# YinkaiYu/Hybrid-Monte-Carlo-for-d-wave-SC

Hardware: AMD Instinct MI355X
Metric: fp64 leapfrog steps/sec at L=32, 1→8 MI355X; % fp64 MFMA roofline (higher is better)
Workload: dtype f64; 1 GPU; L=32 beta=16 single-chain HMC (BASELINE configs[2], C3); L=32, N=1024, bdg_dim=2048, chains_per_gpu=1, Nt=7, therm_sweeps=100, poles=12, parallelism=single GPU

## Files before the change

hybrid-monte-carlo-for-d-wave-sc_amd/csrc/dwhmc_cr_sparse.hip:

```cpp
#include "dwhmc_device.h"
#include "dwhmc_internal.h"

namespace dwh {
namespace {

__device__ __forceinline__ void cmac(double2& a, double2 b, double2 c) {
  a.x = fma(b.x, c.x, fma(-b.y, c.y, a.x));
  a.y = fma(b.x, c.y, fma(b.y, c.x, a.y));
}
__device__ __forceinline__ void rmac(double2& a, double s, double2 c) {
  a.x = fma(s, c.x, a.x);
  a.y = fma(s, c.y, a.y);
}

__device__ __forceinline__ double sp_flip(double x, unsigned m) {
  return __builtin_bit_cast(double, __builtin_bit_cast(unsigned long long, x) ^ ((unsigned long long)m << 32));
}

__device__ __forceinline__ double sp_uniform(double x) {
  const unsigned long long b = __builtin_bit_cast(unsigned long long, x);
  const unsigned lo = __builtin_amdgcn_readfirstlane((unsigned)b), hi = __builtin_amdgcn_readfirstlane((unsigned)(b >> 32));
  return __builtin_bit_cast(double, (unsigned long long)hi << 32 | lo);
}

// ... 6 lines not shown
    crot = cb < HB ? cb + HB : cb - HB;
    mx = cb >= HB ? 0x80000000u : 0u;
    my = cb < HB ? 0x80000000u : 0u;
  }
  __device__ __forceinline__ double2 ld(const double2* base, unsigned row) const {
    return *reinterpret_cast<const double2*>(reinterpret_cast<const char*>(base) + (row + crot));
  }
  __device__ __forceinline__ double2 sign(double2 u) const {
    return make_double2(sp_flip(u.x, mx), sp_flip(u.y, my));
  }
};

__device__ __forceinline__ double2 sp_cval(double2 x, int m) {
  if ((m & 0x3fffff) == 0) return x;
  const int op = (m >> 22) & 3;
  return make_double2(op == 2 ? -0.5 * x.x : 0.5 * x.x, op == 0 ? 0.5 * x.y : -0.5 * x.y);
}

constexpr int kSpRowsWG = 4;
constexpr int NZ = kCrSpNZ, NH = kCrSpNZ - 1;
#ifndef SP_WAVES_F
#define SP_WAVES_F 6
#endif
#ifndef SP_WAVES_B
#define SP_WAVES_B 6
#endif
#ifndef SP_RPW_B
#define SP_RPW_B 1
#endif
template <int BP>
constexpr int kSpWavesF = BP <= 64 ? SP_WAVES_F : 2;
template <int BP>
constexpr int kSpWavesB = BP <= 64 ? SP_WAVES_B : 2;

__device__ __forceinline__ void wave_sync() {
  __builtin_amdgcn_fence(__ATOMIC_RELEASE, "wavefront");
  __builtin_amdgcn_wave_barrier();
  __builtin_amdgcn_fence(__ATOMIC_ACQUIRE, "wavefront");
}

__device__ __forceinline__ double2 sp_ld(const double2* base, unsigned off) {
  return *reinterpret_cast<const double2*>(reinterpret_cast<const char*>(base) + off);
}
__device__ __forceinline__ void sp_st(double2* base, unsigned off, double2 v) {
  *reinterpret_cast<double2*>(reinterpret_cast<char*>(base) + off) = v;
}

template <int BP, int NB>
struct ColStage {
  static constexpr int TOT = NB * NZ * BP, IT = (TOT + 64 * kSpRowsWG - 1) / (64 * kSpRowsWG);
  int m[IT];
  double2 x[IT];
  __device__ __forceinline__ void load_meta(const int* __restrict__ tcm) {
#pragma unroll
    for (int i = 0; i < IT; ++i) m[i] = tcm[min((int)threadIdx.x + 64 * kSpRowsWG * i, TOT - 1)];
  }
  __device__ __forceinline__ void load_values(const double2* __restrict__ tcv, const double2* __restrict__ Dc) {
#pragma unroll
    for (int i = 0; i < IT; ++i) {
      const int q = min((int)threadIdx.x + 64 * kSpRowsWG * i, TOT - 1), s = m[i] & 0x3fffff;
      x[i] = *(s ? Dc + (s - 1) : tcv + q);
    }
  }
  __device__ __forceinline__ void pin_meta() {
#pragma unroll
    for (int i = 0; i < IT; ++i) asm volatile("" : "+v"(m[i]));
// ... 159 lines not shown
#pragma unroll
          for (int e = 0; e < NH; ++e) gh[o][g][e][j] = sp_ld(base, t.ho[o][g][e] + cl[j]);
          gp[o][g][j] = bc.ld(base, t.po[o][g]);
        }
    }
    __builtin_amdgcn_sched_barrier(0);
    double2 yk[NCL][2];
#pragma unroll
    for (int j = 0; j < NCL; ++j) {
      const BotCol<BP> bc(cl[j]);
      double2 ya = make_double2(0.0, 0.0), yc = ya;
#pragma unroll
      for (int o = 0; o < 2; ++o) {
#pragma unroll
        for (int e = 0; e < NH; ++e) {
          rmac(ya, t.hv[o][e], gh[o][0][e][j]);
          rmac(yc, t.hv[o][e], gh[o][1][e][j]);
        }
        cmac(ya, pw[o], bc.sign(gp[o][0][j]));
        cmac(yc, pw[o], bc.sign(gp[o][1][j]));
      }
      yk[j][0] = ya;
      yk[j][1] = yc;
    }
#pragma unroll
    for (int j = 0; j < NCL; ++j)
      asm volatile("" : "+v"(yk[j][0].x), "+v"(yk[j][0].y), "+v"(yk[j][1].x), "+v"(yk[j][1].y));
    __builtin_amdgcn_sched_barrier(0);
    __syncthreads();
    if (i == 0) {
      cs.finish(cv, ci);
      __syncthreads();
    }
#pragma unroll
    for (int j = 0; j < NCL; ++j) {
      const int c = cl[j] / sizeof(double2);
      double2 za = make_double2(0.0, 0.0), zc = za;
#pragma unroll
      for (int e = 0; e < NZ; ++e) {
        const double2 wa = cv[0][e][c], we = cv[1][e][c];
        const unsigned ka = ci[0][e][c], ke = ci[1][e][c];
        cmac(za, sp_ld(gr[w][0], ka), wa);
        cmac(zc, sp_ld(gr[w][1], ka), wa);
        cmac(za, sp_ld(gr[w][2], ke), we);
        cmac(zc, sp_ld(gr[w][3], ke), we);
      }
      if (l + 64 * j < BP) {
        sp_st(base, t.oya + cl[j], yk[j][0]);
        sp_st(base, t.oyc + cl[j], yk[j][1]);
        sp_st(base, t.oza + cl[j], za);
        sp_st(base, t.ozc + cl[j], zc);
      }
    }
    wave_sync();
#pragma unroll
    for (int j = 0; j < NCL; ++j)
      if (l + 64 * j < BP) {
        sp_st(sc[w][0], cl[j], yk[j][0]);
        sp_st(sc[w][1], cl[j], yk[j][1]);
      }
    wave_sync();
#pragma unroll
    for (int j = 0; j < NCL; ++j) {
      const int c = cl[j] / sizeof(double2);
      double2 mx = make_double2(0.0, 0.0);
#pragma unroll
      for (int e = 0; e < NZ; ++e) {
        cmac(mx, sp_ld(sc[w][0], ci[0][e][c]), cv[0][e][c]);
        cmac(mx, sp_ld(sc[w][1], ci[1][e][c]), cv[1][e][c]);
      }
      if (l + 64 * j < BP) sp_st(base, t.omx + cl[j], mx);
    }
    if (RPW > 1) wave_sync();
  }
}

}

void launch_cr_sp_fwd(const CrDims& c, double2* pool, const CrSpRowFwd* recs, int n, const double2* tcv,
                      const int* tcm, const double2* Delta, hipStream_t s) {
  if (n <= 0) return;
  const dim3 g(n * (c.BP / 2 / kSpRowsWG), c.nbatch), b(64 * kSpRowsWG);
  switch (c.BP) {
    case 32: hipLaunchKernelGGL(k_cr_sp_fwd<32>, g, b, 0, s, pool, c.item, recs, tcv, tcm, Delta, 2 * c.N, c.P); break;
    case 64: hipLaunchKernelGGL(k_cr_sp_fwd<64>, g, b, 0, s, pool, c.item, recs, tcv, tcm, Delta, 2 * c.N, c.P); break;
    default: hipLaunchKernelGGL(k_cr_sp_fwd<96>, g, b, 0, s, pool, c.item, recs, tcv, tcm, Delta, 2 * c.N, c.P); break;
  }
}

void launch_cr_sp_bwd(const CrDims& c, double2* pool, const CrSpRowBwd* recs, int n, const double2* tcv,
                      const int* tcm, const double2* Delta, hipStream_t s) {
  if (n <= 0) return;
  constexpr int RPW = SP_RPW_B;
  const dim3 g(n * (c.BP / 2 / (kSpRowsWG * RPW)), c.nbatch), b(64 * kSpRowsWG);
  switch (c.BP) {
    case 32: hipLaunchKernelGGL((k_cr_sp_bwd<32, RPW>), g, b, 0, s, pool, c.item, recs, tcv, tcm, Delta, 2 * c.N, c.P); break;
    case 64: hipLaunchKernelGGL((k_cr_sp_bwd<64, RPW>), g, b, 0, s, pool, c.item, recs, tcv, tcm, Delta, 2 * c.N, c.P); break;
    default: hipLaunchKernelGGL((k_cr_sp_bwd<96, RPW>), g, b, 0, s, pool, c.item, recs, tcv, tcm, Delta, 2 * c.N, c.P); break;
  }
}

}
```

hybrid-monte-carlo-for-d-wave-sc_amd/csrc/dwhmc_internal.h:

```cpp
#pragma once
#include <hip/hip_runtime.h>
#include <stddef.h>
#include <stdint.h>

namespace dwh {

constexpr int kGJ = 64;
constexpr int kSlots = 4;
constexpr int kHSlots = 9;

struct Dims {
  int N;
  int Np;
  int nb;
  int nc;
  int P;
  int nbatch;
  int64_t mat;
  int nld;
};

struct KickDrift {
  double kick, drift, cap;
  int* flag;
// ... 38 lines not shown
#endif
void launch_cr_fill(const CrDims& c, double2* pool, const int* list, int nlist, const int* hcol,
                    const double* hval, const int* Dcol, const int* Dsrc, const double2* Delta,
                    const double* ypole, const int64_t* off_ph, hipStream_t s);
void launch_cr_pair_force(const CrDims& c, double2* pool, const int64_t* bond4, const double* cpole,
                          double2* Delta, double2* Pair, double2* F, double2* Pi,
                          const KickDrift& kd, double beta, double J, hipStream_t s);
void launch_cr_fermion_energy(const CrDims& c, const double2* pool, const int64_t* doff,
                              const double* ldpart, const double* cpole, double Cx, double beta,
                              double* part, unsigned* done, double* Ef, double* Trhh, hipStream_t s);
struct SiteGuard {
  const double2* Delta = nullptr;
  const int* site4 = nullptr;
  double cap4 = 0.0;
  int* flag = nullptr;
};
void launch_cr_inv(const CrDims& c, double2* pool, const int* blk, const int* dst, const int* slot,
                   int n, double* ldpart, hipStream_t s, const SiteGuard& sg = SiteGuard{});
inline bool cr_supported_inv0(int BP) { return BP == 64 || BP == 32 || BP == 96; }
void launch_cr_inv0(const CrDims& c, double2* pool, const int* blk, const int* rblk, const int* dst,
                    const int* slot, int n, double* ldpart, const double* ldA, hipStream_t s,
                    const double2* Delta = nullptr, const int* site4 = nullptr, double cap4 = 0.0,
                    int* flag = nullptr);
inline bool cr_supported_side(int BP) { return BP == 64; }
void launch_cr_inv_side(const CrDims& c, double2* pool, const int* blk, const int* dst, const int* slot,
                        int n, double* ldpart, const CrTask* stasks, int nst, int maxt32, hipStream_t s,
                        const SiteGuard& sg = SiteGuard{});
constexpr int kCrSpNZ = 4;
inline bool cr_supported_sparse0(int BP) { return BP == 32 || BP == 64 || BP == 96; }
struct CrSpFwd {
  int dk, uk, lk, uel, lel, uer, ler, dir, dil, od, ou, ol;
};
struct CrSpBwd {
  int gaa, gac, gca, gcc, ua, le, la, ue, oza, ozc, oya, oyc, omx, pad0, pad1, pad2;
};
struct alignas(256) CrSpRowFwd {
  double hv[3][kCrSpNZ - 1];
  double ps[3];
  uint32_t ho[3][kCrSpNZ - 1];
  uint32_t po[3], pd[3];
  uint32_t dk, od, ou, ol;
};
struct alignas(256) CrSpRowBwd {
  double hv[2][kCrSpNZ - 1];
  double ps[2];
  uint32_t ho[2][2][kCrSpNZ - 1];
  uint32_t po[2][2], pd[2];
  uint32_t g[4];
  uint32_t oza, ozc, oya, oyc, omx;
};
static_assert(sizeof(CrSpRowFwd) == 256 && sizeof(CrSpRowBwd) == 256, "one record: 256 bytes");
void launch_cr_sp_fwd(const CrDims& c, double2* pool, const CrSpRowFwd* recs, int n, const double2* tcv,
                      const int* tcm, const double2* Delta, hipStream_t s);
void launch_cr_sp_bwd(const CrDims& c, double2* pool, const CrSpRowBwd* recs, int n, const double2* tcv,
                      const int* tcm, const double2* Delta, hipStream_t s);
struct CrGemmCfg {
  int ts, ksplit;
};
void launch_cr_gemm(const CrDims& c, double2* pool, const CrTask* tasks, int ntasks, int maxt32,
                    int maxt16, const CrSlot* slots, int nslot_wgs, const CrGemmCfg& cfg, double sg,
                    hipStream_t s);

void launch_fill_hz(const Dims& d, double2* M, const int* hcol, const double* hval,
                    const double* ypole, hipStream_t s);
void launch_gj_pivot(const Dims& d, double2* M, int k, double2* Pout, double2* XRout,
                     double2* colcopy, double2* nextcol, double* ldpart, hipStream_t s);
struct GJPanelPtrs {
  const double2 *CpA, *CpB, *XR1, *XR2, *Pb1, *Pb2;
  double2 *CpBw, *CpN;
};
int gj_update_tiles(const Dims& d, int mode);
void launch_gj_update(const Dims& d, double2* M, int k, int mode, const GJPanelPtrs& p,
                      hipStream_t s);
void launch_dvals(const Dims& d, const int* Dsrc, const double2* Delta, double2* Dv,
                  hipStream_t s);
void launch_assemble(const Dims& d, const double2* R, double2* S, const int* Dcol,
                     const double2* Dv, const int* hcol, const double* hval, const double* ypole,
                     hipStream_t s);
void launch_contract(const Dims& d, const double2* R, const double2* SinvT, const int* Dcol,
                     const double2* Dv, double2* G12nn, double2* diagS, hipStream_t s);
void launch_pair_force(const Dims& d, const double2* G12nn, const int* bond_ij,
                       const int* bond_ji, const double* cpole, double2* Delta, double2* Pair,
// ... 137 lines not shown
```

hybrid-monte-carlo-for-d-wave-sc_amd/csrc/dwhmc_plan.cpp:

```cpp
#include "dwhmc_plan.h"

#include <algorithm>
#include <array>
#include <cstdio>
#include <cstdlib>
#include <cstring>
#include <initializer_list>
#include <set>
#include <string>
#include <utility>

#include "../../include/dwhmc.h"
#include "dwhmc_model.h"

namespace dwh {

namespace {
struct SpRow {
  double hv[dwh::kCrSpNZ - 1] = {};
  int hk[dwh::kCrSpNZ - 1] = {};
  double ps = 0.0;
  int pk = 0, pd = 0;
};
SpRow sp_row(const std::vector<int>& rowpat, int b, int r, int Lx, int Ly, int BP, const std::vector<int>& hcol,
// ... 43 lines not shown
  auto at = [&](int b, int k) { return (uint32_t)(((int64_t)b * HP + k) * BP * (int64_t)sizeof(double2)); };
  auto cols = [&](int cb) {
    for (int k = cb * E; k < (cb + 1) * E; ++k) {
      const int w = pl.colpat[k], op = (w >> 22) & 3, idx = (w >> 14) & 0xff, src = colsrc[k];
      a.cv.push_back(colval[k]);
      a.cm.push_back((src < 0 ? 0 : src + 1) | op << 22 | idx << 24);
    }
  };
  for (const dwh::CrSpFwd& t : pl.sp_fwd) {
    const int sparse[3] = {t.uk, t.ler, t.lel}, dense[3] = {t.dir, t.dir, t.dil};
    for (int r = 0; r < HP; ++r) {
      dwh::CrSpRowFwd q{};
      for (int o = 0; o < 3; ++o) {
        const SpRow s = row(sparse[o], r);
        for (int e = 0; e < NZ - 1; ++e) {
          q.hv[o][e] = -s.hv[e];
          q.ho[o][e] = at(dense[o], s.hk[e]);
        }
        q.ps[o] = -s.ps;
        q.po[o] = at(dense[o], s.pk);
        q.pd[o] = (uint32_t)s.pd;
      }
      q.dk = at(t.dk, r);
      q.od = at(t.od, r);
      q.ou = at(t.ou, r);
      q.ol = at(t.ol, r);
      a.rf.push_back(q);
    }
    cols(t.lk);
    cols(t.uel);
    cols(t.uer);
  }
  a.col_bwd0 = a.cv.size();
  for (const dwh::CrSpBwd& t : pl.sp_bwd) {
    const int sparse[2] = {t.la, t.ue}, dense[2][2] = {{t.gaa, t.gac}, {t.gca, t.gcc}};
    for (int r = 0; r < HP; ++r) {
      dwh::CrSpRowBwd q{};
      for (int o = 0; o < 2; ++o) {
        const SpRow s = row(sparse[o], r);
        for (int g = 0; g < 2; ++g) {
          for (int e = 0; e < NZ - 1; ++e) q.ho[o][g][e] = at(dense[o][g], s.hk[e]);
          q.po[o][g] = at(dense[o][g], s.pk);
        }
        for (int e = 0; e < NZ - 1; ++e) q.hv[o][e] = s.hv[e];
        q.ps[o] = s.ps;
        q.pd[o] = (uint32_t)s.pd;
      }
      q.g[0] = at(t.gaa, r);
      q.g[1] = at(t.gca, r);
      q.g[2] = at(t.gac, r);
      q.g[3] = at(t.gcc, r);
      q.oza = at(t.oza, r);
      q.ozc = at(t.ozc, r);
      q.oya = at(t.oya, r);
      q.oyc = at(t.oyc, r);
      q.omx = at(t.omx, r);
      a.rb.push_back(q);
    }
    cols(t.ua);
    cols(t.le);
  }
  return a;
}

namespace {
bool cr_sparse_patterns(int Lx, int Ly, int BP, const std::vector<int>& hcol, const std::vector<int>& Dcol,
                        std::vector<int>& rowpat, std::vector<int>& colpat) {
  const int HP = BP / 2, NZ = dwh::kCrSpNZ;
  const int empty = 3 << 22;
  rowpat.assign((size_t)3 * Ly * NZ * BP, empty);
  colpat.assign((size_t)3 * Ly * NZ * BP, empty);
  for (int t = 1; t <= 2; ++t)
    for (int y = 0; y < Ly; ++y) {
      if ((t == 1 && Ly < 2) || (t == 2 && Ly < 3)) continue;
      const int b = t * Ly + y;
      const int yr = (t == 2) ? (y + 1) % Ly : y, yc = (t == 1) ? (y + 1) % Ly : y;
      std::set<std::pair<int, int>> top;
      for (int x = 0; x < Lx; ++x) {
        const int i = yr * Lx + x;
        for (int s = 0; s < kHSlots; ++s) {
          const int j = hcol[(size_t)i * kHSlots + s];
          if (j >= 0 && j / Lx == yc) top.insert({x, j % Lx});
        }
        for (int s = 0; s < kSlots; ++s) {
          const int j = Dcol[(size_t)i * kSlots + s];
          if (j >= 0 && j / Lx == yc) top.insert({x, HP + j % Lx});
        }
      }
      std::vector<int> nhop(HP, 0), npair(HP, 0);
// ... 54 lines not shown
int sp_nrow(const std::vector<int>& pat, int b, int r, int BP) {
  int n = 0;
  for (int e = 0; e < dwh::kCrSpNZ; ++e) n += ((pat[((size_t)b * dwh::kCrSpNZ + e) * BP + r] >> 22) & 3) != 3;
  return n;
}
}

int cr_rows_per_block(int64_t Lx, int64_t Ly) {
  auto ok = [&](int64_t r) { return r >= 1 && Ly % r == 0 && dwh::cr_supported_bp((int)(2 * ((r * Lx + 15) / 16 * 16))); };
  int64_t r = std::max<int64_t>(1, 16 / Lx);
  while (r > 1 && !ok(r)) --r;
  return ok(r) ? (int)r : 0;
}

int choose_algo(int32_t algo_req, int64_t Lx, int64_t Ly, AlgoChoice* out) {
  std::string want = "auto";
  if (algo_req == DWH_ALGO_DENSE) want = "dense";
  else if (algo_req == DWH_ALGO_CR) want = "cr";
  else if (algo_req == DWH_ALGO_EIG) want = "eig";
  else if (const char* e = std::getenv("DWHMC_ALGO")) want = e;
  if (want != "auto" && want != "dense" && want != "cr" && want != "eig")
    return fail(nullptr, DWH_ERR_ARG, "DWHMC_ALGO must be auto, dense, cr or eig");
  out->want = want == "dense" ? DWH_ALGO_DENSE : want == "cr" ? DWH_ALGO_CR : want == "eig" ? DWH_ALGO_EIG : DWH_ALGO_AUTO;
  out->cr_ok = cr_rows_per_block(Lx, Ly) > 0;
  out->site_guard = out->want == DWH_ALGO_CR || (out->want == DWH_ALGO_AUTO && out->cr_ok);
  return DWH_OK;
}

CrPlan build_cr_plan(int Lx, int Ly, int BP, const std::vector<int>& Dcol, bool side, int nbatch,
                     int ncu, bool inv0, const std::vector<int>* hcol) {
  constexpr int side_woff = 2, side_m = 4;
  CrPlan pl;
  const int HP = BP / 2;
  const bool sparse0 = [&] {
    const char* e = std::getenv("DWHMC_CR_SPARSE0");
    const bool force = e && *e == '1';
    if ((e && *e == '0') || !hcol || Ly % 2 != 0 || Ly < 4 || !dwh::cr_supported_sparse0(BP)) return false;
    if (!force && BP < 64) return false;
    return cr_sparse_patterns(Lx, Ly, BP, *hcol, Dcol, pl.rowpat, pl.colpat);
  }();
  if (!sparse0) {
    pl.rowpat.clear();
    pl.colpat.clear();
  }
  const int merge_max_m = [&] {
    const char* e = std::getenv("DWHMC_CR_MERGE");
    return e ? std::max(0, std::atoi(e)) : side ? 4 : 8;
  }();
  const bool merge = merge_max_m >= 2;
  auto nr = [&](int b, int r) { return sp_nrow(pl.rowpat, b, r, BP); };
  auto nc = [&](int b, int c) { return sp_nrow(pl.colpat, b, c, BP); };
  int nblk = 3 * Ly;
  std::vector<char> qform(3 * Ly, 0);
  auto nb = [&]() {
    qform.push_back(0);
    return nblk++;
  };
  auto nbq = [&]() {
    qform.push_back(1);
    return nblk++;
  };
  struct Level {
    int m;
    std::vector<int> D, U, L, E, K;
    std::vector<int> Dinv;
    std::vector<int> V1, V2, W1, W2;
    std::vector<char> elim;
    bool sparse = false;
    bool merged = false;
    std::vector<std::array<int, 6>> xa, xc;
// ... 300 lines not shown
              t.bq = qform[src[k][1]] ? 1 : 0;
              merge_tasks.push_back(t);
            }
            return x;
          };
          if (u.elim[a / 2]) f.xa[e] = expand(a / 2, f.V1[e], f.W1[e]);
          if (u.elim[(c / 2) % u.m]) f.xc[e] = expand((c / 2) % u.m, f.V2[e], f.W2[e]);
        }
      }
      if (!side)
        for (const dwh::CrTask& t : merge_tasks) {
          cur_tasks.push_back(t);
          cur_keep.push_back(nullptr);
        }
    }
    flush(1.0);
    if (!ul_tasks.empty()) {
      cur_tasks = ul_tasks;
      cur_keep.assign(ul_tasks.size(), nullptr);
      flush(1.0, true, inv_ord);
    }
    if (side && !merge_tasks.empty()) {
      cur_tasks = merge_tasks;
      cur_keep.assign(merge_tasks.size(), nullptr);
      flush(1.0, true, n_inv - 1);
    }
    levels.push_back(cur);
    cur = nxt;
  }
  const int Dfin = add_inv({cur.D[0]}, slot)[0];
  std::vector<int> GD{Dfin}, GU{Dfin}, GL{Dfin};
  struct GeeTask { int out, cin, a0, b0, a1, b1; };
  std::vector<GeeTask> pend;
  auto emit_pend = [&] {
    for (const GeeTask& t : pend) task(t.out, t.cin, {{t.a0, t.b0}, {t.a1, t.b1}});
    pend.clear();
  };
  for (int li = (int)levels.size() - 1; li >= 0; --li) {
    Level& lv = levels[li];
    if (!pend.empty() && !lv.merged) {
      emit_pend();
      flush(1.0);
    }
    const int m = lv.m, mn = (int)lv.K.size();
    std::vector<int> gd(m, -1), gu(m, -1), gl(m, -1);
    for (int kk = 0; kk < mn; ++kk) {
      const int k = lv.K[kk];
      gd[k] = GD[kk];
      if (!(k + 1 < m && lv.elim[k + 1])) {
        gu[k] = GU[kk];
        gl[k] = GL[kk];
      }
    }
    const bool sel = (li == 0);
    const int H0 = sel ? HP : 0, H1 = sel ? HP + Lx : BP;
    if (lv.sparse) {
      CrStage st{};
      st.kind = 2;
      st.sp = 1;
      st.first = (int)pl.sp_bwd.size();
      struct Bw { int e, a, za, zc, ya, yc, mx; };
      std::vector<Bw> bw;
      for (int e : lv.E) {
        const int a = e - 1, c = (e + 1) % m;
        const int ia = a / 2, ic = (c / 2) % mn;
        const int Gaa = GD[ia], Gcc = GD[ic], Gac = GU[ia], Gca = GL[ia];
        const Bw x{e, a, nbq(), nbq(), nbq(), nbq(), nb()};
        bw.push_back(x);
        pl.sp_bwd.push_back(dwh::CrSpBwd{Gaa, Gac, Gca, Gcc, lv.U[a], lv.L[e], lv.L[a], lv.U[e], x.za, x.zc, x.ya,
                                         x.yc, x.mx, 0, 0, 0});
        for (int cc = 0; cc < BP; ++cc) st.flops += 8.0 * HP * 2 * (nc(lv.U[a], cc) + nc(lv.L[e], cc));
        for (int r = 0; r < HP; ++r) st.flops += 8.0 * BP * 3 * (nr(lv.L[a], r) + nr(lv.U[e], r));
      }
      st.n = (int)pl.sp_bwd.size() - st.first;
      pl.stages.push_back(st);
      std::vector<int> tn(m, -1);
      for (const Bw& x : bw) {
        const int e = x.e, a = x.a, D = lv.Dinv[e];
        const int gea = nb(), gec = nb(), gae = nb(), gce = nb();
        tn[e] = nbq();
        w_c0 = H0;
        w_c1 = H1;
        keep_next = &need[2][a];
        task(gea, -1, {{D, x.ya}});
        keep_next = &need[1][e];
        task(gec, -1, {{D, x.yc}});
        keep_next = &need[1][a];
        task(gae, -1, {{x.za, D}});
        keep_next = &need[2][e];
        task(gce, -1, {{x.zc, D}});
        keep_next = nullptr;
        w_c0 = 0;
        w_c1 = BP;
        task(tn[e], -1, {{D, x.mx}});
        gu[a] = gae;
        gl[a] = gea;
        gu[e] = gec;
        gl[e] = gce;
      }
      flush(-1.0);
      for (int e : lv.E) {
        const int gee = nb();
        keep_next = &need[0][e];
        task(gee, lv.Dinv[e], {{tn[e], lv.Dinv[e]}});
        gd[e] = gee;
      }
      keep_next = nullptr;
      flush(-1.0);
      GD = gd;
      GU = gu;
      GL = gl;
      continue;
    }
    const Level* up = lv.merged ? &levels[li + 1] : nullptr;
    emit_pend();
    lv.Gea.assign(m, -1);
    lv.Gec.assign(m, -1);
    lv.Gae.assign(m, -1);
    lv.Gce.assign(m, -1);
    for (int e : lv.E) {
      const int a = e - 1, c = (e + 1) % m;
      const int ia = a / 2, ic = (c / 2) % mn;
      const int Gaa = GD[ia], Gcc = GD[ic];
      const int Gac = mn == 1 ? GD[0] : GU[ia];
      const int Gca = mn == 1 ? GD[0] : GL[ia];
      const int gea = nb(), gec = nb(), gae = nb(), gce = nb();
      const bool xa = up && lv.xa[e][0] >= 0, xc = up && lv.xc[e][0] >= 0;
      w_c0 = H0;
      w_c1 = H1;
      keep_next = sel ? &need[2][a] : nullptr;
      if (xa) {
// ... 30 lines not shown
      gl[e] = gce;
      lv.Gea[e] = gea;
      lv.Gec[e] = gec;
      lv.Gae[e] = gae;
      lv.Gce[e] = gce;
    }
    flush(1.0);
    const bool defer = li >= 1 && levels[li - 1].merged;
    for (int e : lv.E) {
      if (defer) {
        pend.push_back(GeeTask{lv.Dinv[e], lv.Dinv[e], lv.W1[e], lv.Gae[e], lv.W2[e], lv.Gce[e]});
      } else {
        keep_next = sel ? &need[0][e] : nullptr;
        task(lv.Dinv[e], lv.Dinv[e], {{lv.W1[e], lv.Gae[e]}, {lv.W2[e], lv.Gce[e]}});
      }
      gd[e] = lv.Dinv[e];
    }
    keep_next = nullptr;
    if (!defer) flush(1.0);
    GD = gd;
    GU = gu;
    GL = gl;
  }
  const int N = Lx * Ly;
  const int64_t BB = (int64_t)HP * BP;
  pl.goff.assign((size_t)N * kSlots, -1);
  pl.doff.assign(N, 0);
  for (int i = 0; i < N; ++i) {
    const int x = i % Lx, y = i / Lx;
    for (int s = 0; s < kSlots; ++s) {
      const int j = Dcol[(size_t)i * kSlots + s];
      if (j < 0) continue;
      const int xj = j % Lx, yj = j / Lx;
      int blk;
      if (Ly == 1 || yj == y) blk = GD[y];
      else if (yj == (y + 1) % Ly) blk = GU[y];
      else blk = GL[(y - 1 + Ly) % Ly];
      pl.goff[(size_t)i * kSlots + s] = blk * BB + (int64_t)x * BP + (HP + xj);
    }
    pl.doff[i] = GD[y] * BB + (int64_t)x * BP + x;
  }
  std::vector<char> rewrite(3 * Ly, 0);
  for (int b = 0; b < 3 * Ly; ++b) {
    pl.fill_all.push_back(b);
    if (rewrite[b]) pl.fill_step.push_back(b);
  }
  pl.off_ph.assign((size_t)N * kSlots, -1);
  auto blk_of = [&](int yr, int yc) {
    if (yc == yr) return yr;
    if (Ly >= 2 && yc == (yr + 1) % Ly) return Ly + yr;
    return 2 * Ly + yc;
  };
  for (int i = 0; i < N; ++i)
    for (int s = 0; s < kSlots; ++s) {
      const int j = Dcol[(size_t)i * kSlots + s];
      if (j < 0) continue;
      const int yi = i / Lx, xi = i % Lx, yj = j / Lx, xj = j % Lx;
      const int b = blk_of(yi, yj);
      if (rewrite[b]) continue;
      pl.off_ph[(size_t)i * kSlots + s] = b * BB + (int64_t)xi * BP + (HP + xj);
      pl.n_ph++;
    }
  pl.nblk = nblk;
  return pl;
}

CrGemmCfg cr_gemm_config(const CrDims& c, int ntiles16) {
  const CrGemmCfg forced = [] {
    CrGemmCfg f{0, 1};
    if (const char* e = std::getenv("DWHMC_CR_GEMM")) {
      f.ts = std::atoi(e);
// ... 129 lines not shown
      nnn[0 * N + i] = idx(x + 1, y + 1);
      nnn[1 * N + i] = idx(x - 1, y + 1);
      nnn[2 * N + i] = idx(x - 1, y - 1);
      nnn[3 * N + i] = idx(x + 1, y - 1);
    }
  const std::vector<double> clean((size_t)N, 0.0);
  HostModel m;
  if (int rc = build_host_model(Lx, Ly, 1.0, -0.35, 0.0, nn.data(), nnn.data(), 1, clean.data(), &m, false)) return rc;
  return plan_cr(Lx, Ly, 1, (int)nbatch, m.Dcol, m.hcol, side != 0, inv0 != 0, 256, c, pl);
}
}

}

using namespace dwh;

extern "C" {

int dwh_debug_cr_plan_check(int64_t Lx, int64_t Ly, int64_t nbatch, int32_t side, int32_t inv0, int64_t* stats) {
  CrDims c;
  CrPlan pl;
  if (int rc = plan_periodic(Lx, Ly, nbatch, side, inv0, &c, &pl)) return rc;
  const int Lyc = c.Ly, BP = c.BP;
  cr_plan_dump(pl, nbatch, false);
  std::vector<int> written(pl.nblk, -1);
  for (int b = 0; b < 3 * Lyc && b < pl.nblk; ++b) written[b] = -2;
  for (int r : pl.inv0_r) written[r] = -2;
  int64_t nside = 0, ninv = 0, ngemm = 0, ntask = 0;
  char buf[256];
  const int ntc = BP / 16;
  std::set<std::pair<int, int>> tiles_written;
  std::vector<char> whole(pl.nblk, 0);
  for (int b = 0; b < pl.nblk; ++b) whole[b] = written[b] == -2;
  for (int si = 0; si < (int)pl.stages.size(); ++si) {
    const CrStage& st = pl.stages[si];
    if (st.kind == 0) {
      for (int k = 0; k < st.n; ++k) whole[pl.inv_dst[st.first + k]] = 1;
      for (int k = 0; k < st.ntiles; ++k) whole[pl.tasks[st.tfirst + k].out] = 1;
    } else if (st.kind == 2) {
      for (int k = 0; k < st.n; ++k) {
        if (st.sp == 0) {
          const dwh::CrSpFwd& t = pl.sp_fwd[st.first + k];
          whole[t.od] = whole[t.ou] = whole[t.ol] = 1;
        } else {
          const dwh::CrSpBwd& t = pl.sp_bwd[st.first + k];
          whole[t.oza] = whole[t.ozc] = whole[t.oya] = whole[t.oyc] = whole[t.omx] = 1;
        }
      }
    } else {
      for (int k = 0; k < st.ntiles; ++k) {
        const dwh::CrTile& t = pl.tiles16[st.tfirst + k];
        tiles_written.insert({t.out, t.tr * ntc + t.tc});
      }
    }
    std::vector<std::pair<int, int>> rd;
    std::vector<std::pair<int, int>> wr;
    auto add_task = [&](const dwh::CrTask& t, int id) {
      for (int h = 0; h < t.nt; ++h) {
        rd.push_back({t.a[h], id + (1 << 20)});
        rd.push_back({t.b[h], id + (1 << 20)});
      }
      if (t.cin >= 0) rd.push_back({t.cin, id});
      wr.push_back({t.out, id});
    };
    if (st.kind == 0) {
      ++ninv;
      for (int k = 0; k < st.n; ++k) {
        rd.push_back({pl.inv_blk[st.first + k], -1 - k});
        wr.push_back({pl.inv_dst[st.first + k], -1 - k});
      }
      if (st.ntiles > 0) ++nside;
      for (int k = 0; k < st.ntiles; ++k) add_task(pl.tasks[st.tfirst + k], k);
    } else if (st.kind == 2) {
      ++ngemm;
      for (int k = 0; k < st.n; ++k) {
        const int id = k + (1 << 21);
        if (st.sp == 0) {
          const dwh::CrSpFwd& t = pl.sp_fwd[st.first + k];
          for (int b : {t.dk, t.uk, t.lk, t.uel, t.lel, t.uer, t.ler, t.dir, t.dil}) rd.push_back({b, id});
          for (int b : {t.od, t.ou, t.ol}) wr.push_back({b, id});
        } else {
          const dwh::CrSpBwd& t = pl.sp_bwd[st.first + k];
          for (int b : {t.gaa, t.gac, t.gca, t.gcc, t.ua, t.le, t.la, t.ue}) rd.push_back({b, id});
          for (int b : {t.oza, t.ozc, t.oya, t.oyc, t.omx}) wr.push_back({b, id});
        }
      }
    } else {
      ++ngemm;
      for (int k = 0; k < st.n; ++k) add_task(pl.tasks[st.first + k], k);
    }
    ntask += (int64_t)wr.size();
    for (const auto& r : rd) {
      if (r.first < 0 || r.first >= pl.nblk || written[r.first] == -1) {
        std::snprintf(buf, sizeof buf, "stage %d reads block %d before any stage writes it", si, r.first);
        return fail(nullptr, DWH_ERR_STATE, buf);
      }
      for (const auto& w : wr)
        if (w.first == r.first && w.second != r.second) {
          std::snprintf(buf, sizeof buf, "stage %d reads block %d that the same stage writes", si, r.first);
          return fail(nullptr, DWH_ERR_STATE, buf);
        }
    }
    for (size_t i = 0; i < wr.size(); ++i)
      for (size_t j = i + 1; j < wr.size(); ++j)
        if (wr[i].first == wr[j].first && wr[i].second != wr[j].second) {
          std::snprintf(buf, sizeof buf, "stage %d writes block %d from two tasks", si, wr[i].first);
          return fail(nullptr, DWH_ERR_STATE, buf);
        }
    for (const auto& w : wr) {
      if (w.first >= 0 && w.first < pl.nblk && written[w.first] == -2) {
        std::snprintf(buf, sizeof buf, "stage %d overwrites static block %d", si, w.first);
        return fail(nullptr, DWH_ERR_STATE, buf);
      }
      if (w.first >= 0 && w.first < pl.nblk && written[w.first] == -1) written[w.first] = si;
    }
  }
  const int64_t BB = (int64_t)(BP / 2) * BP;
  auto tile_ok = [&](int64_t o) {
    const int b = (int)(o / BB), r = (int)((o % BB) / BP), col = (int)(o % BP);
    return whole[b] || tiles_written.count({b, (r / 16) * ntc + col / 16}) > 0;
  };
  for (int64_t o : pl.goff)
    if (o >= 0 && (written[o / BB] == -1 || !tile_ok(o)))
      return fail(nullptr, DWH_ERR_STATE, "force gather reads an unwritten block / tile");
  for (int64_t o : pl.doff)
    if (written[o / BB] == -1 || !tile_ok(o)) return fail(nullptr, DWH_ERR_STATE, "E_f gather reads an unwritten block / tile");
  if (stats) {
    stats[0] = (int64_t)pl.stages.size();
    stats[1] = ninv;
    stats[2] = nside;
    stats[3] = ngemm;
    stats[4] = ntask;
    stats[5] = pl.nblk;
  }
  return DWH_OK;
}

int dwh_debug_cr_plan_flops(int64_t Lx, int64_t Ly, int64_t nbatch, int32_t side, int32_t inv0, double* flops) {
  if (!flops) return fail(nullptr, DWH_ERR_ARG, "bad lattice / batch / output");
  CrDims c;
  CrPlan pl;
  if (int rc = plan_periodic(Lx, Ly, nbatch, side, inv0, &c, &pl)) return rc;
  const int BP = c.BP;
  const double bp3 = 8.0 * BP * (double)BP * BP;
  flops[0] = flops[1] = flops[2] = 0.0;
  for (const CrStage& st : pl.stages) {
    if (st.kind == 0) {
      flops[0] += st.n * bp3;
      flops[2] += st.flops;
    } else {
      flops[1] += st.flops;
    }
// ... 6 lines not shown
```

hybrid-monte-carlo-for-d-wave-sc_amd/csrc/dwhmc_plan.h:

```cpp
#pragma once
#include <cstdint>
#include <vector>

#include "dwhmc_internal.h"

namespace dwh {

struct CrStage {
  int kind;
  int first, n;
  double sg;
  double flops;
  int maxt32, maxt16, ntmax;
  int tfirst, ntiles;
  dwh::CrGemmCfg cfg;
  int sfirst = 0, nswg = 0;
  int l0 = 0;
  int sp = 0;
};

struct CrPlan {
  int nblk = 0;
  std::vector<CrStage> stages;
  std::vector<dwh::CrTask> tasks;
  std::vector<dwh::CrTile> tiles16;
  std::vector<dwh::CrSlot> slots;
  std::vector<int> inv_blk, inv_dst, inv_slot;
  std::vector<int> inv0_r;
  std::vector<int64_t> goff, doff;
  std::vector<int> fill_all, fill_step;
  std::vector<int64_t> off_ph;
  int n_ph = 0;
  std::vector<dwh::CrSpFwd> sp_fwd;
  std::vector<dwh::CrSpBwd> sp_bwd;
  std::vector<int> rowpat, colpat;
};

struct SpTaskArrays {
  std::vector<dwh::CrSpRowFwd> rf;
  std::vector<dwh::CrSpRowBwd> rb;
  std::vector<int> cm;
  std::vector<double2> cv;
  size_t col_bwd0 = 0;
};

SpTaskArrays cr_sparse_task_arrays(const CrPlan& pl, int Lx, int Ly, int BP, const std::vector<int>& hcol,
                                   const std::vector<double>& hval, const std::vector<int>& Dcol,
                                   const std::vector<int>& Dsrc);
void cr_sparse_colvals(const std::vector<int>& colpat, int Lx, int Ly, int BP, const std::vector<int>& hcol,
                       const std::vector<double>& hval, const std::vector<int>& Dcol, const std::vector<int>& Dsrc,
                       std::vector<double2>& colval, std::vector<int>& colsrc);
int cr_rows_per_block(int64_t Lx, int64_t Ly);

struct AlgoChoice {
  int32_t want = 0;
  bool cr_ok = false, site_guard = false;
};
int choose_algo(int32_t algo_req, int64_t Lx, int64_t Ly, AlgoChoice* out);

constexpr int kCrFromEnv = -1;
int plan_cr(int64_t Lx, int64_t Ly, int P, int nbatch, const std::vector<int>& Dcol, const std::vector<int>& hcol,
            int side, int inv0, int ncu, CrDims* c, CrPlan* pl);
void cr_plan_dump(const CrPlan& pl, int64_t nbatch, bool cfg);

}
```

Baseline: 4176 leapfrog steps/s.

## Compute only needed inter-row bond Green entries inside sparse backward kernel

Instead of writing the full z_a/z_c blocks and then running four dense GEMM tasks to form G_ae and G_ce, the sparse backward kernel now dot-products z with the matching Dinv row in-register. It reduces the products with DPP/shuffle reductions and stores only the per-row bond entries the force gather needs into a compact bond area. The plan drops the two GEMM tasks per level, records per-row bond columns and offsets, and points force gather offsets at the bond area. This removes two dense block GEMMs and their block writes per eliminated level. The cost is extra loads and reductions in the sparse kernel, and a new requirement that each row have a unique inter-row bond column.

Measured after the change: 4179 leapfrog steps/s (median of 5 runs). No clear change (+0.1%).

```diff
diff --git a/hybrid-monte-carlo-for-d-wave-sc_amd/csrc/dwhmc_cr_sparse.hip b/hybrid-monte-carlo-for-d-wave-sc_amd/csrc/dwhmc_cr_sparse.hip
--- a/hybrid-monte-carlo-for-d-wave-sc_amd/csrc/dwhmc_cr_sparse.hip
+++ b/hybrid-monte-carlo-for-d-wave-sc_amd/csrc/dwhmc_cr_sparse.hip
@@ -62,6 +62,14 @@
 constexpr int kSpWavesF = BP <= 64 ? SP_WAVES_F : 2;
 template <int BP>
 constexpr int kSpWavesB = BP <= 64 ? SP_WAVES_B : 2;
+
+__device__ __forceinline__ double sp_sum16(double x) {
+  x += __builtin_amdgcn_update_dpp(x, x, 0xB1, 0xf, 0xf, true);
+  x += __builtin_amdgcn_update_dpp(x, x, 0x4E, 0xf, 0xf, true);
+  x += __builtin_amdgcn_update_dpp(x, x, 0x141, 0xf, 0xf, true);
+  x += __builtin_amdgcn_update_dpp(x, x, 0x140, 0xf, 0xf, true);
+  return x;
+}
 
 __device__ __forceinline__ void wave_sync() {
   __builtin_amdgcn_fence(__ATOMIC_RELEASE, "wavefront");
@@ -287,6 +295,7 @@
       cs.finish(cv, ci);
       __syncthreads();
     }
+    double2 zk[NCL][2], dv[NCL][2];
 #pragma unroll
     for (int j = 0; j < NCL; ++j) {
       const int c = cl[j] / sizeof(double2);
@@ -300,17 +309,28 @@
         cmac(za, sp_ld(gr[w][2], ke), we);
         cmac(zc, sp_ld(gr[w][3], ke), we);
       }
+      zk[j][0] = za;
+      zk[j][1] = zc;
+    }
+#pragma unroll
+    for (int j = 0; j < NCL; ++j)
+      asm volatile("" : "+v"(zk[j][0].x), "+v"(zk[j][0].y), "+v"(zk[j][1].x), "+v"(zk[j][1].y));
+    __builtin_amdgcn_sched_barrier(0);
+#pragma unroll
+    for (int j = 0; j < NCL; ++j) {
+      const unsigned k = cl[j] / sizeof(double2);
+      unsigned bk = (k < HP ? k * BP + HP : (k - HP) * BP) * (unsigned)sizeof(double2);
+      asm volatile("" : "+v"(bk));
+      dv[j][0] = sp_ld(base, t.bd[0] + bk);
+      dv[j][1] = sp_ld(base, t.bd[1] + bk);
+    }
+    __builtin_amdgcn_sched_barrier(0);
+    wave_sync();
+#pragma unroll
+    for (int j = 0; j < NCL; ++j)
       if (l + 64 * j < BP) {
         sp_st(base, t.oya + cl[j], yk[j][0]);
         sp_st(base, t.oyc + cl[j], yk[j][1]);
-        sp_st(base, t.oza + cl[j], za);
-        sp_st(base, t.ozc + cl[j], zc);
-      }
-    }
-    wave_sync();
-#pragma unroll
-    for (int j = 0; j < NCL; ++j)
-      if (l + 64 * j < BP) {
         sp_st(sc[w][0], cl[j], yk[j][0]);
         sp_st(sc[w][1], cl[j], yk[j][1]);
       }
@@ -325,6 +345,25 @@
         cmac(mx, sp_ld(sc[w][1], ci[1][e][c]), cv[1][e][c]);
       }
       if (l + 64 * j < BP) sp_st(base, t.omx + cl[j], mx);
+    }
+    __builtin_amdgcn_sched_barrier(0);
+    {
+      double2 pa = make_double2(0.0, 0.0), pc = pa;
+#pragma unroll
+      for (int j = 0; j < NCL; ++j) {
+        const unsigned fx = l + 64 * j < HP ? 0x80000000u : 0u;
+        const double2 wa = l + 64 * j < BP ? zk[j][0] : make_double2(0.0, 0.0);
+        const double2 wc = l + 64 * j < BP ? zk[j][1] : make_double2(0.0, 0.0);
+        cmac(pa, wa, make_double2(sp_flip(dv[j][0].x, fx), -dv[j][0].y));
+        cmac(pc, wc, make_double2(sp_flip(dv[j][1].x, fx), -dv[j][1].y));
+      }
+      const bool hi = l & 32, odd = l & 16;
+      const double2 keep = hi ? pc : pa, send = hi ? pa : pc;
+      const double2 h = make_double2(keep.x + __shfl_xor(send.x, 32, 64), keep.y + __shfl_xor(send.y, 32, 64));
+      const double v = sp_sum16((odd ? h.y : h.x) + __shfl_xor(odd ? h.x : h.y, 16, 64));
+      const unsigned o = hi ? t.bo[1] : t.bo[0];
+      if ((l & 15) == 0 && o != kCrNone)
+        *reinterpret_cast<double*>(reinterpret_cast<char*>(base) + (o + (odd ? 8u : 0u))) = v;
     }
     if (RPW > 1) wave_sync();
   }
diff --git a/hybrid-monte-carlo-for-d-wave-sc_amd/csrc/dwhmc_internal.h b/hybrid-monte-carlo-for-d-wave-sc_amd/csrc/dwhmc_internal.h
--- a/hybrid-monte-carlo-for-d-wave-sc_amd/csrc/dwhmc_internal.h
+++ b/hybrid-monte-carlo-for-d-wave-sc_amd/csrc/dwhmc_internal.h
@@ -94,7 +94,7 @@
   int dk, uk, lk, uel, lel, uer, ler, dir, dil, od, ou, ol;
 };
 struct CrSpBwd {
-  int gaa, gac, gca, gcc, ua, le, la, ue, oza, ozc, oya, oyc, omx, pad0, pad1, pad2;
+  int gaa, gac, gca, gcc, ua, le, la, ue, dinv, oya, oyc, omx, pad0, pad1, pad2, pad3;
 };
 struct alignas(256) CrSpRowFwd {
   double hv[3][kCrSpNZ - 1];
@@ -109,7 +109,8 @@
   uint32_t ho[2][2][kCrSpNZ - 1];
   uint32_t po[2][2], pd[2];
   uint32_t g[4];
-  uint32_t oza, ozc, oya, oyc, omx;
+  uint32_t oya, oyc, omx;
+  uint32_t bd[2], bo[2];
 };
 static_assert(sizeof(CrSpRowFwd) == 256 && sizeof(CrSpRowBwd) == 256, "one record: 256 bytes");
 void launch_cr_sp_fwd(const CrDims& c, double2* pool, const CrSpRowFwd* recs, int n, const double2* tcv,
diff --git a/hybrid-monte-carlo-for-d-wave-sc_amd/csrc/dwhmc_plan.cpp b/hybrid-monte-carlo-for-d-wave-sc_amd/csrc/dwhmc_plan.cpp
--- a/hybrid-monte-carlo-for-d-wave-sc_amd/csrc/dwhmc_plan.cpp
+++ b/hybrid-monte-carlo-for-d-wave-sc_amd/csrc/dwhmc_plan.cpp
@@ -99,7 +99,8 @@
     cols(t.uer);
   }
   a.col_bwd0 = a.cv.size();
-  for (const dwh::CrSpBwd& t : pl.sp_bwd) {
+  for (size_t ti = 0; ti < pl.sp_bwd.size(); ++ti) {
+    const dwh::CrSpBwd& t = pl.sp_bwd[ti];
     const int sparse[2] = {t.la, t.ue}, dense[2][2] = {{t.gaa, t.gac}, {t.gca, t.gcc}};
     for (int r = 0; r < HP; ++r) {
       dwh::CrSpRowBwd q{};
@@ -117,11 +118,14 @@
       q.g[1] = at(t.gca, r);
       q.g[2] = at(t.gac, r);
       q.g[3] = at(t.gcc, r);
-      q.oza = at(t.oza, r);
-      q.ozc = at(t.ozc, r);
       q.oya = at(t.oya, r);
       q.oyc = at(t.oyc, r);
       q.omx = at(t.omx, r);
+      for (int w = 0; w < 2; ++w) {
+        const int pj = pl.sp_bcol[(ti * 2 + w) * HP + r];
+        q.bd[w] = at(t.dinv, 0) + (uint32_t)(std::max(pj, 0) * sizeof(double2));
+        q.bo[w] = pj < 0 ? dwh::kCrNone : (uint32_t)(cr_bond_off(pl, BP, (int)ti, w, r) * (int64_t)sizeof(double2));
+      }
       a.rb.push_back(q);
     }
     cols(t.ua);
@@ -242,10 +246,24 @@
   constexpr int side_woff = 2, side_m = 4;
   CrPlan pl;
   const int HP = BP / 2;
+  std::vector<std::vector<std::vector<int>>> bcol(2, std::vector<std::vector<int>>(Ly, std::vector<int>(HP, -1)));
+  bool bcol_ok = true;
+  if (Ly >= 3)
+    for (int i = 0; i < Lx * Ly; ++i) {
+      const int pi = i % Lx, y = i / Lx;
+      for (int s = 0; s < kSlots; ++s) {
+        const int j = Dcol[(size_t)i * kSlots + s];
+        if (j < 0 || j / Lx == y) continue;
+        const int pj = j % Lx, yj = j / Lx;
+        int& b = yj == (y + 1) % Ly ? bcol[0][y][pi] : bcol[1][(y - 1 + Ly) % Ly][pi];
+        if (b >= 0 && b != pj) bcol_ok = false;
+        b = pj;
+      }
+    }
   const bool sparse0 = [&] {
     const char* e = std::getenv("DWHMC_CR_SPARSE0");
     const bool force = e && *e == '1';
-    if ((e && *e == '0') || !hcol || Ly % 2 != 0 || Ly < 4 || !dwh::cr_supported_sparse0(BP)) return false;
+    if ((e && *e == '0') || !hcol || Ly % 2 != 0 || Ly < 4 || !dwh::cr_supported_sparse0(BP) || !bcol_ok) return false;
     if (!force && BP < 64) return false;
     return cr_sparse_patterns(Lx, Ly, BP, *hcol, Dcol, pl.rowpat, pl.colpat);
   }();
@@ -612,6 +630,7 @@
   std::vector<int> GD{Dfin}, GU{Dfin}, GL{Dfin};
   struct GeeTask { int out, cin, a0, b0, a1, b1; };
   std::vector<GeeTask> pend;
+  std::vector<int> bond_u(Ly, -1), bond_l(Ly, -1);
   auto emit_pend = [&] {
     for (const GeeTask& t : pend) task(t.out, t.cin, {{t.a0, t.b0}, {t.a1, t.b1}});
     pend.clear();
@@ -639,25 +658,36 @@
       st.kind = 2;
       st.sp = 1;
       st.first = (int)pl.sp_bwd.size();
-      struct Bw { int e, a, za, zc, ya, yc, mx; };
+      struct Bw { int e, a, ya, yc, mx; };
       std::vector<Bw> bw;
       for (int e : lv.E) {
         const int a = e - 1, c = (e + 1) % m;
         const int ia = a / 2, ic = (c / 2) % mn;
         const int Gaa = GD[ia], Gcc = GD[ic], Gac = GU[ia], Gca = GL[ia];
-        const Bw x{e, a, nbq(), nbq(), nbq(), nbq(), nb()};
+        const Bw x{e, a, nbq(), nbq(), nb()};
         bw.push_back(x);
-        pl.sp_bwd.push_back(dwh::CrSpBwd{Gaa, Gac, Gca, Gcc, lv.U[a], lv.L[e], lv.L[a], lv.U[e], x.za, x.zc, x.ya,
-                                         x.yc, x.mx, 0, 0, 0});
+        const int ti = (int)pl.sp_bwd.size();
+        pl.sp_bwd.push_back(dwh::CrSpBwd{Gaa, Gac, Gca, Gcc, lv.U[a], lv.L[e], lv.L[a], lv.U[e], lv.Dinv[e], x.ya,
+                                         x.yc, x.mx, 0, 0, 0, 0});
         for (int cc = 0; cc < BP; ++cc) st.flops += 8.0 * HP * 2 * (nc(lv.U[a], cc) + nc(lv.L[e], cc));
         for (int r = 0; r < HP; ++r) st.flops += 8.0 * BP * 3 * (nr(lv.L[a], r) + nr(lv.U[e], r));
+        pl.sp_bcol.insert(pl.sp_bcol.end(), bcol[0][a].begin(), bcol[0][a].end());
+        pl.sp_bcol.insert(pl.sp_bcol.end(), bcol[1][e].begin(), bcol[1][e].end());
+        for (int r = 0; r < HP; ++r) st.flops += 8.0 * BP * ((bcol[0][a][r] >= 0) + (bcol[1][e][r] >= 0));
+        bond_u[a] = 2 * ti;
+        bond_l[e] = 2 * ti + 1;
       }
       st.n = (int)pl.sp_bwd.size() - st.first;
       pl.stages.push_back(st);
+      pl.bond_nblk = (int)((2 * (int64_t)HP * st.n + (int64_t)HP * BP - 1) / ((int64_t)HP * BP));
+      for (int k = 0; k < pl.bond_nblk; ++k) {
+        const int b = nb();
+        if (k == 0) pl.bond_blk = b;
+      }
       std::vector<int> tn(m, -1);
       for (const Bw& x : bw) {
         const int e = x.e, a = x.a, D = lv.Dinv[e];
-        const int gea = nb(), gec = nb(), gae = nb(), gce = nb();
+        const int gea = nb(), gec = nb();
         tn[e] = nbq();
         w_c0 = H0;
         w_c1 = H1;
@@ -665,18 +695,12 @@
         task(gea, -1, {{D, x.ya}});
         keep_next = &need[1][e];
         task(gec, -1, {{D, x.yc}});
-        keep_next = &need[1][a];
-        task(gae, -1, {{x.za, D}});
-        keep_next = &need[2][e];
-        task(gce, -1, {{x.zc, D}});
         keep_next = nullptr;
         w_c0 = 0;
         w_c1 = BP;
         task(tn[e], -1, {{D, x.mx}});
-        gu[a] = gae;
         gl[a] = gea;
         gu[e] = gec;
-        gl[e] = gce;
       }
       flush(-1.0);
       for (int e : lv.E) {
@@ -773,11 +797,12 @@
       const int j = Dcol[(size_t)i * kSlots + s];
       if (j < 0) continue;
       const int xj = j % Lx, yj = j / Lx;
-      int blk;
+      int blk, bond = -1;
       if (Ly == 1 || yj == y) blk = GD[y];
-      else if (yj == (y + 1) % Ly) blk = GU[y];
-      else blk = GL[(y - 1 + Ly) % Ly];
-      pl.goff[(size_t)i * kSlots + s] = blk * BB + (int64_t)x * BP + (HP + xj);
+      else if (yj == (y + 1) % Ly) blk = GU[y], bond = bond_u[y];
+      else blk = GL[(y - 1 + Ly) % Ly], bond = bond_l[(y - 1 + Ly) % Ly];
+      pl.goff[(size_t)i * kSlots + s] =
+          bond >= 0 ? cr_bond_off(pl, BP, bond / 2, bond % 2, x) : blk * BB + (int64_t)x * BP + (HP + xj);
     }
     pl.doff[i] = GD[y] * BB + (int64_t)x * BP + x;
   }
@@ -973,6 +998,7 @@
   std::set<std::pair<int, int>> tiles_written;
   std::vector<char> whole(pl.nblk, 0);
   for (int b = 0; b < pl.nblk; ++b) whole[b] = written[b] == -2;
+  std::set<int64_t> bond_written;
   for (int si = 0; si < (int)pl.stages.size(); ++si) {
     const CrStage& st = pl.stages[si];
     if (st.kind == 0) {
@@ -985,7 +1011,13 @@
           whole[t.od] = whole[t.ou] = whole[t.ol] = 1;
         } else {
           const dwh::CrSpBwd& t = pl.sp_bwd[st.first + k];
-          whole[t.oza] = whole[t.ozc] = whole[t.oya] = whole[t.oyc] = whole[t.omx] = 1;
+          whole[t.oya] = whole[t.oyc] = whole[t.omx] = 1;
+          for (int w = 0; w < 2; ++w)
+            for (int r = 0; r < BP / 2; ++r)
+              if (pl.sp_bcol[((size_t)(st.first + k) * 2 + w) * (BP / 2) + r] >= 0 &&
+                  !bond_written.insert(cr_bond_off(pl, BP, st.first + k, w, r)).second)
+                return fail(nullptr, DWH_ERR_STATE, "sparse backward stage writes a bond entry twice");
+          for (int b = 0; b < pl.bond_nblk; ++b) written[pl.bond_blk + b] = si;
         }
       }
     } else {
@@ -1022,8 +1054,8 @@
           for (int b : {t.od, t.ou, t.ol}) wr.push_back({b, id});
         } else {
           const dwh::CrSpBwd& t = pl.sp_bwd[st.first + k];
-          for (int b : {t.gaa, t.gac, t.gca, t.gcc, t.ua, t.le, t.la, t.ue}) rd.push_back({b, id});
-          for (int b : {t.oza, t.ozc, t.oya, t.oyc, t.omx}) wr.push_back({b, id});
+          for (int b : {t.gaa, t.gac, t.gca, t.gcc, t.ua, t.le, t.la, t.ue, t.dinv}) rd.push_back({b, id});
+          for (int b : {t.oya, t.oyc, t.omx}) wr.push_back({b, id});
         }
       }
     } else {
@@ -1032,6 +1064,10 @@
     }
     ntask += (int64_t)wr.size();
     for (const auto& r : rd) {
+      if (r.first >= pl.bond_blk && r.first < pl.bond_blk + pl.bond_nblk) {
+        std::snprintf(buf, sizeof buf, "stage %d reads bond-area block %d", si, r.first);
+        return fail(nullptr, DWH_ERR_STATE, buf);
+      }
       if (r.first < 0 || r.first >= pl.nblk || written[r.first] == -1) {
         std::snprintf(buf, sizeof buf, "stage %d reads block %d before any stage writes it", si, r.first);
         return fail(nullptr, DWH_ERR_STATE, buf);
@@ -1059,6 +1095,7 @@
   const int64_t BB = (int64_t)(BP / 2) * BP;
   auto tile_ok = [&](int64_t o) {
     const int b = (int)(o / BB), r = (int)((o % BB) / BP), col = (int)(o % BP);
+    if (b >= pl.bond_blk && b < pl.bond_blk + pl.bond_nblk) return bond_written.count(o) > 0;
     return whole[b] || tiles_written.count({b, (r / 16) * ntc + col / 16}) > 0;
   };
   for (int64_t o : pl.goff)
diff --git a/hybrid-monte-carlo-for-d-wave-sc_amd/csrc/dwhmc_plan.h b/hybrid-monte-carlo-for-d-wave-sc_amd/csrc/dwhmc_plan.h
--- a/hybrid-monte-carlo-for-d-wave-sc_amd/csrc/dwhmc_plan.h
+++ b/hybrid-monte-carlo-for-d-wave-sc_amd/csrc/dwhmc_plan.h
@@ -34,7 +34,13 @@
   std::vector<dwh::CrSpFwd> sp_fwd;
   std::vector<dwh::CrSpBwd> sp_bwd;
   std::vector<int> rowpat, colpat;
+  int bond_blk = -1, bond_nblk = 0;
+  std::vector<int> sp_bcol;
 };
+inline int64_t cr_bond_off(const CrPlan& pl, int BP, int ti, int w, int r) {
+  const int HP = BP / 2;
+  return (int64_t)pl.bond_blk * HP * BP + ((int64_t)ti * 2 + w) * HP + r;
+}
 
 struct SpTaskArrays {
   std::vector<dwh::CrSpRowFwd> rf;
```
